# dpeerlab/segger

Hardware: AMD Instinct MI355X
Metric: edges scored/sec (tx->cell) fwd+bwd (higher is better)
Workload: dtype bf16; 1 GPU; C2: single Xenium-scale tile per GPU, 1000000 tx, 10000 nuclei, k=15 kNN (Ett=15000000, Etb=393796, Ep=2435646), training step fwd+bwd+Adam, attention dropout 0.2; parallelism=dp1

## Files before the change

include/segger_amd.h:

```cpp
#ifndef SEGGER_AMD_H
#define SEGGER_AMD_H

#include <stddef.h>
#include <stdint.h>

#ifdef __cplusplus
extern "C" {
#endif

#if defined(__GNUC__) || defined(__clang__)
#pragma GCC visibility push(default)
#endif

#define SEGGER_ABI_VERSION 32

enum segger_status {
  SEGGER_OK = 0,
  SEGGER_EINVAL = -1,
  SEGGER_EUNSUPPORTED = -2,
  SEGGER_EHIP = -3,
  SEGGER_EWORKSPACE = -4
};

enum segger_dtype { SEGGER_F32 = 0, SEGGER_BF16 = 1, SEGGER_F16 = 2 };
// ... 90 lines not shown
  int64_t ld_gxr;
  float* grad_att;
  float* grad_bias;
  void* workspace;
  size_t workspace_bytes;
  const uint8_t* keep_bits_dst;
  const uint8_t* keep_bits_src;
  int32_t src_unique;
  void* zero_rows_out;
  int64_t ld_zero;
  int32_t grad_xl_zeroed;
  int32_t passes;
} segger_gatv2_bwd_args;

size_t segger_gatv2_bwd_workspace_bytes(int64_t n_dst, int32_t heads, int32_t channels);
int segger_gatv2_bwd(const segger_gatv2_bwd_args* args, segger_stream_t stream);
int segger_gatv2_bwd_pair(const segger_gatv2_bwd_args* a, const segger_gatv2_bwd_args* b, segger_stream_t stream);
int segger_dropout_bits(const int32_t* eid, int64_t n_edges, int32_t heads, float dropout_p, const uint64_t* seeds,
                        int32_t n_seeds, const uint64_t* seed_dev, uint8_t* bits, int64_t plane_stride,
                        segger_stream_t stream);
typedef struct segger_bits_job {
  const int32_t* eid;
  int64_t n_edges;
  const uint64_t* seeds;
  int32_t n_seeds;
  int32_t reserved_;
  uint8_t* bits;
  int64_t plane_stride;
} segger_bits_job;
int segger_dropout_bits_many(const segger_bits_job* jobs, int32_t n_jobs, int32_t heads, float dropout_p,
// ... 458 lines not shown
```

segger_amd/_lib.py:

```python
from __future__ import annotations

import ctypes as C
import os
from typing import Optional

import torch

_HERE = os.path.dirname(os.path.abspath(__file__))
LIB_PATH = os.environ.get("SEGGER_AMD_LIB") or os.path.join(_HERE, "libsegger_amd.so")
ABI_VERSION = 32
THRESHOLDS_CHUNK = 1024
FEATURES_TILE, FEATURES_SLAB_ROWS, FEATURES_MAX_SLABS = 64, 512, 32
FEATURES_MAX_COLS, FEATURES_MAX_K = 32768, 256
KNN_BF_MAX_D, KNN_BF_MAX_K, KNN_BF_MAX_SLABS = 256, 64, 32
CONTAM_MAX_TYPES, CONTAM_MAX_K, CONTAM_MAX_REF_GENES, CONTAM_LDS_BYTES = 256, 64, 32768, 65536
MORPH_MAX_VERTS, MORPH_COLS, MORPH_ERR_OFFSETS, MORPH_ERR_CAP = 4096, 12, 1, 2
PJOIN_CONTAINS, PJOIN_INTERSECTS = 0, 1
PJOIN_ERR_OFFSETS, PJOIN_ERR_CAP, PJOIN_ERR_BUFFER, PJOIN_ERR_FILL = 1, 2, 4, 8
BOUNDARY_MAX_SMOOTHING, BOUNDARY_CHUNK_MAX_HULL, BOUNDARY_COUNTERS = 6, 2048, 8
OUTLINE_MAX_POINTS, OUTLINE_COUNTERS = 2048, 10

SEGGER_F32, SEGGER_BF16, SEGGER_F16 = 0, 1, 2
DTYPE_CODE = {torch.float32: SEGGER_F32, torch.bfloat16: SEGGER_BF16, torch.float16: SEGGER_F16}

# ... 187 lines not shown
class WgradArgs(C.Structure):
    _fields_ = [("dy", vp), ("ld_dy", C.c_int64), ("x", vp), ("ld_x", C.c_int64), ("w_t", vp), ("n_rows", C.c_int64),
                ("m_out", C.c_int32), ("reserved_", C.c_int32), ("grad_w", vp), ("grad_b", vp), ("dx", vp),
                ("ld_dx", C.c_int64), ("workspace", vp), ("workspace_bytes", C.c_size_t)]


EXPORTS = {
    "segger_abi_version": (C.c_int, []),
    "segger_csr_block_tables": (C.c_int, [vp, vp, vp, C.c_int64, C.c_int64, vp, vp, vp, vp, vp]),
    "segger_last_error": (C.c_char_p, []),
    "segger_csr_from_coo_workspace_bytes": (C.c_size_t, [C.c_int64, C.c_int64]),
    "segger_csr_from_coo": (C.c_int, [vp, vp, C.c_int64, C.c_int64, C.c_int64, vp, vp, vp, vp, vp, C.c_size_t, vp]),
    "segger_csr_row_order": (C.c_int, [vp, C.c_int64, C.c_int32, vp, vp]),
    "segger_gatv2_fwd": (C.c_int, [C.POINTER(GatFwdArgs), vp]),
    "segger_gatv2_bwd_workspace_bytes": (C.c_size_t, [C.c_int64, C.c_int32, C.c_int32]),
    "segger_gatv2_bwd": (C.c_int, [C.POINTER(GatBwdArgs), vp]),
    "segger_dropout_bits": (C.c_int, [vp, C.c_int64, C.c_int32, C.c_float, vp, C.c_int32, vp, vp, C.c_int64, vp]),
    "segger_gatv2_has_specialised": (C.c_int, [C.c_int32, C.c_int32]),
    "segger_coo_unique": (C.c_int, [vp, C.c_int64, C.c_int64, vp, vp, vp]),
    "segger_stage": (C.c_int, [C.POINTER(StageSeg), C.c_int32, vp]),
    "segger_adam_step": (C.c_int, [C.POINTER(AdamTensor), C.c_int32, C.c_double, C.c_double, C.c_double, C.c_double, vp]),
    "segger_adam_step_ex": (C.c_int, [C.POINTER(AdamTensor), C.c_int32, C.c_double, C.c_double, C.c_double, C.c_double, C.c_int32, vp, C.c_int64, vp]),
    "segger_adam_step_dev": (C.c_int, [C.POINTER(AdamTensor), C.c_int32, vp, C.c_int32, vp, C.c_int64, vp]),
    "segger_transpose_many": (C.c_int, [C.POINTER(TransposeSeg), C.c_int32, vp]),
    "segger_posmlp_supported": (C.c_int, [C.c_int32, C.c_int32, C.c_int32]),
    "segger_posmlp_fwd": (C.c_int, [vp, vp, vp, vp, C.c_int64, C.c_float, C.c_float, vp, vp, vp, vp, vp, vp, vp, vp, vp,
                                    C.c_int32, C.c_int32, vp]),
    "segger_posmlp_wgrad": (C.c_int, [vp, C.c_int64, vp, C.c_int64, C.c_float, C.c_int32, vp, vp, vp, C.c_size_t, vp]),
    "segger_sample_negatives": (C.c_int, [vp, C.c_int64, C.c_int64, vp, C.c_uint64, vp, vp, vp]),
    "segger_edge_cos_argmax": (C.c_int, [C.POINTER(EdgeArgmaxArgs), vp]),
# ... 217 lines not shown
```

segger_amd/csrc/common.h:

```cpp
#pragma once
#include <hip/hip_runtime.h>
#include <stdint.h>
#include <stdio.h>
#include <stdarg.h>
#include "../../include/segger_amd.h"

namespace segger {

void set_error(const char* fmt, ...);
int hip_fail(hipError_t e, const char* what);

#define SEGGER_REQUIRE(cond, ...)                 \
  do {                                            \
    if (!(cond)) {                                \
      ::segger::set_error(__VA_ARGS__);           \
      return SEGGER_EINVAL;                       \
    }                                             \
  } while (0)

#define SEGGER_HIP(call)                                        \
  do {                                                          \
    hipError_t _e = (call);                                     \
    if (_e != hipSuccess) return ::segger::hip_fail(_e, #call); \
  } while (0)
// ... 46 lines not shown
int plan_fwd(const FwdRequest& q, FwdPlan* plan);
int launch_fwd_f32(const FwdRequest& q, const FwdPlan& plan, hipStream_t stream);
int launch_fwd_f32_split(const FwdRequest& q, const FwdPlan& plan, hipStream_t stream);

size_t wgrad_f32_workspace_bytes(int64_t n_rows, int m_out, int k_in);
bool wgrad_f32_split_shape_ok(int m, int k);
int64_t wgrad_f32_split_grid(int64_t n_rows, int m, int k);
int wgrad_f32_split_launch(const float* dy, int64_t ld_dy, const float* x, int64_t ld_x, int64_t n_rows, int m_out, int k_in,
                           float* partial, int64_t* n_slabs, hipStream_t stream);
int wgrad_f32_launch(const void* dy, int64_t ld_dy, const void* x, int64_t ld_x, int64_t n_rows, int m_out, int k_in,
                     float* partial, int64_t* n_slabs, hipStream_t stream);

struct ReduceSeg {
  const float* partial; int64_t n_slabs; int64_t width; int64_t split; float* out0; float* out1;
  float* scratch;
};
constexpr int kReduceGroups = 32;
bool defer_reduce(const ReduceSeg& seg, hipStream_t stream);

constexpr int kWave = 64;
constexpr int kNumXcd = 8;

struct bf16_t { uint16_t v; };
struct f16_t  { uint16_t v; };

#ifdef SEGGER_SCALAR_PAIRS
struct f32x2 {
  float x, y;
};
__device__ __forceinline__ f32x2 operator+(f32x2 a, f32x2 b) { return f32x2{a.x + b.x, a.y + b.y}; }
// ... 160 lines not shown
```

segger_amd/csrc/gatv2.hip:

```cpp
#include "gatv2_launch.h"
#include "draws.h"
#include "post_common.h"

namespace segger {

constexpr int kSlabSplits = 128;

__global__ __launch_bounds__(256) void slab_reduce_stage1(const float* __restrict__ slab, int64_t nblocks, int width,
                                                         float* __restrict__ part) {
  __shared__ float sm[4][64];
  const int lane = threadIdx.x & 63, wave = threadIdx.x >> 6;
  const int colx = blockIdx.x * 64 + lane;
  const int64_t per = (nblocks + kSlabSplits - 1) / kSlabSplits;
  const int64_t r0 = (int64_t)blockIdx.y * per;
  const int64_t r1 = r0 + per < nblocks ? r0 + per : nblocks;
  float s = 0.f;
  if (colx < width)
    for (int64_t r = r0 + wave; r < r1; r += 4) s += slab[r * width + colx];
  sm[wave][lane] = s;
  __syncthreads();
  if (wave == 0 && colx < width) part[(int64_t)blockIdx.y * width + colx] = sm[0][lane] + sm[1][lane] + sm[2][lane] + sm[3][lane];
}

__global__ __launch_bounds__(256) void slab_reduce_stage2(const float* __restrict__ part, int width, int hc,
                                                         float* __restrict__ grad_att, float* __restrict__ grad_bias) {
  const int colx = blockIdx.x * 256 + threadIdx.x;
  if (colx >= width) return;
  float t = 0.f;
  for (int r = 0; r < kSlabSplits; ++r) t += part[(int64_t)r * width + colx];
  if (colx < hc) grad_att[colx] = t;
  else if (grad_bias) grad_bias[colx - hc] = t;
}

// ... 126 lines not shown
                   use_wave_per_row(b->by_dst) && !a->alpha && !b->alpha;
  if (!one) {
    if (!ea) CHECK_RC(launch(Pass::Fwd, pa, a->dtype, a->heads, a->channels, use_wave_per_row(a->by_dst), (hipStream_t)stream));
    if (!eb) CHECK_RC(launch(Pass::Fwd, pb, b->dtype, b->heads, b->channels, use_wave_per_row(b->by_dst), (hipStream_t)stream));
    return SEGGER_OK;
  }
  switch (a->dtype) {
    case SEGGER_F32:  return gatv2_launch_fwd_pair_f32(pa, pb, a->heads, a->channels, (hipStream_t)stream);
    case SEGGER_BF16: return gatv2_launch_fwd_pair_bf16(pa, pb, a->heads, a->channels, (hipStream_t)stream);
    case SEGGER_F16:  return gatv2_launch_fwd_pair_f16(pa, pb, a->heads, a->channels, (hipStream_t)stream);
  }
  set_error("gatv2: unknown dtype %d", a->dtype);
  return SEGGER_EINVAL;
}

extern "C" size_t segger_gatv2_bwd_workspace_bytes(int64_t n_dst, int32_t heads, int32_t channels) {
  if (n_dst <= 0 || heads <= 0 || channels <= 0) return 16;
  const int64_t per = 4 * (int64_t)bwd_row_iters(n_dst);
  const int64_t blocks = (n_dst + per - 1) / per + kNumXcd;
  return (size_t)(blocks + kSlabSplits) * 2 * heads * channels * sizeof(float);
}

namespace {
struct BwdState {
  GatParams p;
  bool direct = false, specialised = false;
  int64_t n_dst = 0, n_src = 0, n_edges = 0;
};

int bwd_prepare(const segger_gatv2_bwd_args* a, BwdState& s) {
  SEGGER_REQUIRE(a != nullptr, "segger_gatv2_bwd: args is NULL");
  SEGGER_REQUIRE(a->heads > 0 && a->channels > 0, "segger_gatv2_bwd: heads/channels must be positive");
  const int hc = a->heads * a->channels;
  const bool specialised = gatv2_has_specialised(a->heads, a->channels);
  g_need_align = specialised;
  CHECK_RC(check_csr("by_dst", a->by_dst));
  const bool direct = a->src_unique != 0;
  SEGGER_REQUIRE(!direct || specialised, "segger_gatv2_bwd: src_unique needs a specialised (heads, channels) geometry");
  if (!direct) {
    CHECK_RC(check_csr("by_src", a->by_src));
    SEGGER_REQUIRE(a->by_dst.n_edges == a->by_src.n_edges && a->by_dst.n_rows == a->by_src.n_cols &&
                   a->by_dst.n_cols == a->by_src.n_rows, "segger_gatv2_bwd: by_dst and by_src describe different graphs");
// ... 5 lines not shown
  if (n_dst > 0) {
    CHECK_RC(check_rows("x_r", a->x_r, a->ld_xr, a->dtype, hc));
    CHECK_RC(check_rows("grad_out", a->grad_out, a->ld_go, a->dtype, hc));
    CHECK_RC(check_rows("pre", a->pre, a->ld_pre, a->dtype, hc));
    CHECK_RC(check_rows("grad_pre", a->grad_pre, a->ld_gp, a->dtype, hc));
    CHECK_RC(check_rows("grad_xr", a->grad_xr, a->ld_gxr, a->dtype, hc));
    SEGGER_REQUIRE(a->lse && a->dsum, "segger_gatv2_bwd: lse / dsum is NULL");
  }
  if (n_src > 0) {
    CHECK_RC(check_rows("x_l", a->x_l, a->ld_xl, a->dtype, hc));
    CHECK_RC(check_rows("grad_xl", a->grad_xl, a->ld_gxl, a->dtype, hc));
  }
  SEGGER_REQUIRE(!(a->dropout_p > 0.f) || n_edges == 0 ||
                     ((a->by_dst.eid || a->keep_bits_dst) && (direct || a->by_src.eid || a->keep_bits_src)),
                 "segger_gatv2_bwd: eid arrays (or keep_bits) are required for dropout");
  const size_t need = segger_gatv2_bwd_workspace_bytes(n_dst, a->heads, a->channels);
  if (a->workspace == nullptr || a->workspace_bytes < need) {
    set_error("segger_gatv2_bwd: workspace %zu < %zu bytes", a->workspace_bytes, need);
    return SEGGER_EWORKSPACE;
  }
  SEGGER_REQUIRE(!a->zero_rows_out || (!direct && specialised),
                 "segger_gatv2_bwd: zero_rows_out needs the two-pass backward of a specialised geometry");
  if (a->zero_rows_out && n_src > 0) CHECK_RC(check_rows("zero_rows_out", a->zero_rows_out, a->ld_zero, a->dtype, hc));

  s.direct = direct; s.specialised = specialised; s.n_dst = n_dst; s.n_src = n_src; s.n_edges = n_edges;
  GatParams& p = s.p;
  p = GatParams{};
  p.xl = a->x_l; p.ld_xl = a->ld_xl; p.xr = a->x_r; p.ld_xr = a->ld_xr;
  p.att = a->att; p.bias = a->bias;
  p.pre = const_cast<void*>(a->pre); p.ld_pre = a->ld_pre; p.lse = const_cast<float*>(a->lse);
  p.gout = a->grad_out; p.ld_go = a->ld_go; p.gpre = a->grad_pre; p.ld_gp = a->ld_gp; p.dsum = a->dsum;
  p.gxl = a->grad_xl; p.ld_gxl = a->ld_gxl; p.gxr = a->grad_xr; p.ld_gxr = a->ld_gxr;
  p.slab = static_cast<float*>(a->workspace);
  p.slope = a->negative_slope; p.apply_gelu = a->apply_gelu;
  set_dropout(p, a->dropout_p, a->seed, a->seed_dev);
  return SEGGER_OK;
}

void bwd_dst_params(const segger_gatv2_bwd_args* a, BwdState& s) {
  GatParams& p = s.p;
  p.indptr = a->by_dst.indptr; p.col = a->by_dst.col; p.eid = a->by_dst.eid; p.order = a->by_dst.row_order;
  p.n_rows = s.n_dst; p.n_edges = s.n_edges; p.rows_per_wave_iter = bwd_row_iters(s.n_dst);
  p.bits = a->keep_bits_dst;
  p.direct_gxl = s.direct ? 1 : 0;
  p.zero_rows = nullptr; p.ld_zero = 0;
}

void bwd_src_params(const segger_gatv2_bwd_args* a, BwdState& s) {
// ... 6 lines not shown
}

int bwd_zero_fill(const segger_gatv2_bwd_args* a, const BwdState& s, hipStream_t stream) {
  const size_t es = esize(a->dtype);
  const int64_t pieces = (int64_t)a->heads * a->channels * es / 16, total = s.n_src * pieces;
  hipLaunchKernelGGL(zero_rows_kernel, dim3((unsigned)((total + 255) / 256)), dim3(256), 0, stream,
                     static_cast<char*>(a->grad_xl), (int64_t)a->ld_gxl * (int64_t)es, pieces, total);
  SEGGER_LAUNCH_CHECK("zero_rows_kernel");
  return SEGGER_OK;
}

int bwd_reduce_slab(const segger_gatv2_bwd_args* a, const BwdState& s, hipStream_t stream) {
  if (!s.specialised) return SEGGER_OK;
  const GatParams& p = s.p;
  const int hc = a->heads * a->channels, width = 2 * hc;
  float* part = p.slab + p.nblocks * width;
  if (defer_reduce(ReduceSeg{p.slab, p.nblocks, width, hc, a->grad_att, a->grad_bias, part}, stream)) return SEGGER_OK;
  hipLaunchKernelGGL(slab_reduce_stage1, dim3((width + 63) / 64, kSlabSplits), dim3(256), 0, stream,
                     p.slab, p.nblocks, width, part);
  hipLaunchKernelGGL(slab_reduce_stage2, dim3((width + 255) / 256), dim3(256), 0, stream,
                     part, width, hc, a->grad_att, a->grad_bias);
  SEGGER_LAUNCH_CHECK("slab_reduce kernels");
  return SEGGER_OK;
}

int bwd_no_destinations(const segger_gatv2_bwd_args* a, hipStream_t stream) {
  const int hc = a->heads * a->channels;
  SEGGER_HIP(hipMemsetAsync(a->grad_att, 0, hc * sizeof(float), stream));
  if (a->grad_bias) SEGGER_HIP(hipMemsetAsync(a->grad_bias, 0, hc * sizeof(float), stream));
  return SEGGER_OK;
}

int64_t bwd_pair_max_rows() {
  static const int64_t v = [] {
    const char* e = getenv("SEGGER_BWD_PAIR_MAX_ROWS");
    return e ? (int64_t)atoll(e) : (int64_t)SEGGER_BWD_PAIR_MAX_ROWS;
// ... 1 lines not shown
  return v;
}
}

extern "C" int segger_gatv2_bwd(const segger_gatv2_bwd_args* a, segger_stream_t stream_) {
  hipStream_t stream = (hipStream_t)stream_;
  BwdState s;
  CHECK_RC(bwd_prepare(a, s));
  SEGGER_REQUIRE(a->passes >= 0 && a->passes <= 3, "segger_gatv2_bwd: passes must be 0 (both), 1 (destination), 2 (source) or 3");
  if (a->passes != 2) {
    bwd_dst_params(a, s);
    if (s.direct && s.n_src > 0 && !a->grad_xl_zeroed) CHECK_RC(bwd_zero_fill(a, s, stream));
    if (s.n_dst > 0) {
      GenericOut gen; gen.grad_att = a->grad_att; gen.grad_bias = a->grad_bias;
      CHECK_RC(launch(Pass::BwdDst, s.p, a->dtype, a->heads, a->channels, use_wave_per_row(a->by_dst), stream, gen));
      if (a->passes != 3) CHECK_RC(bwd_reduce_slab(a, s, stream));
    } else {
      CHECK_RC(bwd_no_destinations(a, stream));
    }
  }
  if (s.direct || a->passes == 1 || a->passes == 3) return SEGGER_OK;
  bwd_src_params(a, s);
  if (s.n_src > 0) CHECK_RC(launch(Pass::BwdSrc, s.p, a->dtype, a->heads, a->channels, use_wave_per_row(a->by_src), stream));
  return SEGGER_OK;
}

extern "C" int segger_gatv2_bwd_pair(const segger_gatv2_bwd_args* a, const segger_gatv2_bwd_args* b, segger_stream_t stream_) {
  hipStream_t stream = (hipStream_t)stream_;
  BwdState sa, sb;
  CHECK_RC(bwd_prepare(a, sa));
  CHECK_RC(bwd_prepare(b, sb));
  const bool zero_by_a = a->zero_rows_out ? (a->zero_rows_out == b->grad_xl && a->ld_zero == b->ld_gxl && b->grad_xl_zeroed)
                                          : !b->grad_xl_zeroed;
  const bool one = !sa.direct && sb.direct && a->dtype == b->dtype && a->heads == b->heads && a->channels == b->channels &&
                   sa.specialised && sa.n_dst > 0 && sa.n_src > 0 && sb.n_dst > 0 && sb.n_src > 0 && sa.n_dst == sb.n_src &&
                   !use_wave_per_row(a->by_dst) && !use_wave_per_row(a->by_src) && use_wave_per_row(b->by_dst) &&
                   zero_by_a && sa.n_src <= bwd_pair_max_rows();
  if (!one) {
    CHECK_RC(segger_gatv2_bwd(a, stream_));
    return segger_gatv2_bwd(b, stream_);
  }
  bwd_dst_params(a, sa);
  sa.p.zero_rows = b->grad_xl; sa.p.ld_zero = b->ld_gxl;
  CHECK_RC(launch(Pass::BwdDst, sa.p, a->dtype, a->heads, a->channels, false, stream));
  CHECK_RC(bwd_reduce_slab(a, sa, stream));
  bwd_src_params(a, sa);
  sa.p.zero_rows = nullptr; sa.p.ld_zero = 0;
  bwd_dst_params(b, sb);
  switch (a->dtype) {
    case SEGGER_F32:  CHECK_RC(gatv2_launch_bwd_src_dst_pair_f32(sa.p, sb.p, a->heads, a->channels, stream)); break;
    case SEGGER_BF16: CHECK_RC(gatv2_launch_bwd_src_dst_pair_bf16(sa.p, sb.p, a->heads, a->channels, stream)); break;
    case SEGGER_F16:  CHECK_RC(gatv2_launch_bwd_src_dst_pair_f16(sa.p, sb.p, a->heads, a->channels, stream)); break;
    default: set_error("gatv2: unknown dtype %d", a->dtype); return SEGGER_EINVAL;
  }
  return bwd_reduce_slab(b, sb, stream);
}

extern "C" int segger_gatv2_has_specialised(int32_t heads, int32_t channels) {
  return gatv2_has_specialised(heads, channels) ? 1 : 0;
}

extern "C" int segger_dropout_bits(const int32_t* eid, int64_t n_edges, int32_t heads, float dropout_p,
                                   const uint64_t* seeds, int32_t n_seeds, const uint64_t* seed_dev, uint8_t* bits,
                                   int64_t plane_stride, segger_stream_t stream) {
  SEGGER_REQUIRE(n_edges >= 0 && heads > 0 && heads <= 8, "segger_dropout_bits: heads must be in 1..8");
  SEGGER_REQUIRE(n_seeds > 0 && n_seeds <= 16 && seeds, "segger_dropout_bits: 1..16 seeds");
  SEGGER_REQUIRE(dropout_p >= 0.f && dropout_p < 1.f, "segger_dropout_bits: dropout_p must be in [0,1)");
  if (n_edges == 0) return SEGGER_OK;
  SEGGER_REQUIRE(eid && bits, "segger_dropout_bits: NULL pointer");
// ... 62 lines not shown
```

segger_amd/csrc/gatv2_kernels.h:

```cpp
#pragma once
#include "common.h"

namespace segger {

#ifndef SEGGER_FWD_UNROLL
#define SEGGER_FWD_UNROLL 4
#endif
#ifndef SEGGER_FWD_UNROLL_WPR
#define SEGGER_FWD_UNROLL_WPR 2
#endif
#ifndef SEGGER_DST_UNROLL
#define SEGGER_DST_UNROLL 4
#endif
#ifndef SEGGER_SRC_UNROLL
#define SEGGER_SRC_UNROLL 4
#endif

#ifndef SEGGER_FWD_WAVES
#define SEGGER_FWD_WAVES 4
#endif
#ifndef SEGGER_BWD_DST_WAVES
#define SEGGER_BWD_DST_WAVES 3
#endif
#ifndef SEGGER_BWD_SRC_WAVES
// ... 24 lines not shown
  const void* xl; int64_t ld_xl;
  const void* xr; int64_t ld_xr;
  const float* att;
  const float* bias;
  void* out; int64_t ld_out;
  void* pre; int64_t ld_pre;
  float* lse;
  float* alpha;
  const void* gout; int64_t ld_go;
  void* gpre; int64_t ld_gp;
  float* dsum;
  void* zero_rows; int64_t ld_zero;
  void* gxl; int64_t ld_gxl;
  void* gxr; int64_t ld_gxr;
  float* slab;
  float slope;
  float drop_scale;
  uint32_t drop_thr;
  uint32_t seed_lo, seed_hi;
  const uint64_t* seed_dev;
  uint64_t seed_raw;
  int32_t apply_gelu;
  int32_t direct_gxl;
  int32_t rows_per_wave_iter;
  int64_t nblocks, nblocks_padded;
};

template <int N, typename F>
__device__ __forceinline__ void static_for(F&& f) {
  if constexpr (N > 0) {
// ... 455 lines not shown
  const LaneGeo L = lane_geo<G>();
  const int h = L.h, ch0 = L.ch0;
  const bool head_leader = L.lane_on && (L.gl % LPH) == 0;
  const char* __restrict__ xl = static_cast<const char*>(p.xl) + (size_t)ch0 * sizeof(T);
  const uint32_t ld_xl = (uint32_t)(p.ld_xl * sizeof(T));
  const bool dropout = p.drop_thr != 0;
  uint32_t seed_lo = p.seed_lo, seed_hi = p.seed_hi;
  if (dropout && p.seed_dev) {
    const uint64_t mixed = splitmix64(p.seed_raw + *p.seed_dev);
    seed_lo = (uint32_t)mixed; seed_hi = (uint32_t)(mixed >> 32);
  }
  constexpr int RPW = WPR ? 1 : NG;
  char* __restrict__ gxl_base = static_cast<char*>(p.gxl) + (size_t)ch0 * sizeof(T);
  const uint32_t ld_gxl = (uint32_t)(p.ld_gxl * sizeof(T));

  f32x2 a1[4], na1[4], a2[4], Pt[4], Qt[4], dbias[4];
  load_att(p.att, ch0, p.slope, kLog2e, a1, a2);
#pragma unroll
  for (int i = 0; i < 4; ++i) { na1[i] = -a1[i]; Pt[i] = splat(0.f); Qt[i] = splat(0.f); dbias[i] = splat(0.f); }

#pragma unroll 1
  for (int it = 0; it < p.rows_per_wave_iter; ++it) {
    const int64_t rbase = ((blk * (int64_t)p.rows_per_wave_iter + it) * 4 + L.wave) * RPW;
    if (rbase >= p.n_rows) break;
    const int64_t pos = rbase + (WPR ? 0 : L.grp);
    const bool row_ok = pos < p.n_rows;
    const int row = visit_row<WPR>(p.order, pos, row_ok);
    int ch0r = L.ch0;
    asm volatile("" : "+v"(ch0r));
    const int ch0 = ch0r;

    f32x2 nxr[4], g[4], Sg[4];
    float D = 0.f, lse = 0.f, Sde = 0.f;
    int64_t beg = 0, end = 0;
// ... 54 lines not shown
        float a_eff = a;
        if constexpr (META != kMetaNone) {
          const bool keep = META == kMetaBits ? (ed[u] & hbit) != 0
                                              : dropout_keep((uint32_t)ed[u], H, h, seed_lo, seed_hi, p.drop_thr);
          da = keep ? da * p.drop_scale : 0.f;
          a_eff = keep ? a * p.drop_scale : 0.f;
        }
        const float de = a * (da - D);
        Sde += de;
        const float nde = -de;
        const f32x2 nde2 = splat(nde);
        f32x2 gx[4];
#pragma unroll
        for (int i = 0; i < 4; ++i) {
          const f32x2 sg = f32x2{sign_mul(nde, nt[i].x), sign_mul(nde, nt[i].y)};
          Pt[i] = pk_fma(nde2, nt[i], Pt[i]);
          Qt[i] = pk_fma(-sg, nt[i], Qt[i]);
          Sg[i] = Sg[i] + sg;
          if constexpr (DIRECT)
            gx[i] = pk_fma(splat(a_eff), g[i], (a1[i] * de + a2[i] * sg) * kLn2);
        }
        if constexpr (DIRECT) {
          if (valid[u] && L.lane_on)
            store_pairs(reinterpret_cast<T*>(gxl_base + (uint64_t)(uint32_t)nbr[u] * ld_gxl), gx);
        }
      }
    };
    if (dropout && p.bits)
      walk_row<GS, WPR, kMetaBits, U>(p.col, p.bits, beg, end, L.lane, L.grp, L.gl, body);
    else if (dropout)
      walk_row<GS, WPR, kMetaEid, U>(p.col, p.eid, beg, end, L.lane, L.grp, L.gl, body);
    else
      walk_row<GS, WPR, kMetaNone, U>(p.col, nullptr, beg, end, L.lane, L.grp, L.gl, body);

    if constexpr (WPR) {
#pragma unroll
      for (int off = GS; off < 64; off <<= 1) {
        Sde += __shfl_xor(Sde, off, 64);
#pragma unroll
        for (int i = 0; i < 4; ++i) {
          Sg[i].x += __shfl_xor(Sg[i].x, off, 64);
          Sg[i].y += __shfl_xor(Sg[i].y, off, 64);
        }
      }
    }
    if (writer) {
      f32x2 dxr[4];
#pragma unroll
      for (int i = 0; i < 4; ++i) dxr[i] = (a1[i] * Sde + a2[i] * Sg[i]) * kLn2;
      store_pairs(static_cast<T*>(p.gxr) + row * p.ld_gxr + ch0, dxr);
    }
  }

  const float c1 = 0.5f * (1.f + p.slope), c2 = 0.5f * (1.f - p.slope);
  float datt[8], db[8];
#pragma unroll
  for (int i = 0; i < 4; ++i) {
    datt[2 * i] = c1 * Pt[i].x + c2 * Qt[i].x; datt[2 * i + 1] = c1 * Pt[i].y + c2 * Qt[i].y;
    db[2 * i] = dbias[i].x; db[2 * i + 1] = dbias[i].y;
  }
#pragma unroll
  for (int off = GS; off < 64; off <<= 1) {
#pragma unroll
    for (int k = 0; k < 8; ++k) {
      datt[k] += __shfl_xor(datt[k], off, 64);
      db[k] += __shfl_xor(db[k], off, 64);
    }
  }
  if (L.grp == 0 && L.lane_on) {
#pragma unroll
    for (int k = 0; k < 8; ++k) { red[L.wave][0][ch0 + k] = datt[k]; red[L.wave][1][ch0 + k] = db[k]; }
  }
  __syncthreads();
  for (int i = threadIdx.x; i < 2 * HC; i += 256) {
    const int which = i / HC, c = i % HC;
    p.slab[blk * (2 * HC) + i] = red[0][which][c] + red[1][which][c] + red[2][which][c] + red[3][which][c];
  }
}

template <typename T, int H, int LPH, bool WPR, bool DIRECT>
__global__ __launch_bounds__(256, DIRECT ? 2 : SEGGER_BWD_DST_WAVES) void gatv2_bwd_dst_kernel(GatParams p) {
  gatv2_bwd_dst_body<T, H, LPH, WPR, DIRECT>(p, blockIdx.x);
}

template <typename T, int H, int LPH, bool WPR>
__device__ __forceinline__ void gatv2_bwd_src_body(SEGGER_BODY_PARAM p, int64_t bid) {
  using G = Geo<H, LPH>;
  constexpr int GS = G::GS, NG = G::NG, U = SEGGER_SRC_UNROLL < GS ? SEGGER_SRC_UNROLL : GS;
  const int64_t blk = xcd_remap(bid, p.nblocks_padded, p.nblocks);
  if (blk < 0) return;
  const LaneGeo L = lane_geo<G>();
  const int h = L.h, ch0 = L.ch0;
  const int64_t pos = WPR ? (blk * 4 + L.wave) : ((blk * 4 + L.wave) * NG + L.grp);
  const bool row_ok = pos < p.n_rows;
  const int row = visit_row<WPR>(p.order, pos, row_ok);
  const char* __restrict__ xr_base = static_cast<const char*>(p.xr) + (size_t)ch0 * sizeof(T);
  const char* __restrict__ g_base = static_cast<const char*>(p.gpre) + (size_t)ch0 * sizeof(T);
  const uint32_t ld_xr = (uint32_t)(p.ld_xr * sizeof(T)), ld_gp = (uint32_t)(p.ld_gp * sizeof(T));
  const bool dropout = p.drop_thr != 0;
  uint32_t seed_lo = p.seed_lo, seed_hi = p.seed_hi;
  if (dropout && p.seed_dev) {
    const uint64_t mixed = splitmix64(p.seed_raw + *p.seed_dev);
    seed_lo = (uint32_t)mixed; seed_hi = (uint32_t)(mixed >> 32);
  }

  f32x2 a1[4], na1[4], a2[4], nv[4], acc[4], Sg[4];
#pragma unroll
  for (int i = 0; i < 4; ++i) { nv[i] = splat(0.f); acc[i] = splat(0.f); Sg[i] = splat(0.f); }
  float Sde = 0.f;
  int64_t beg = 0, end = 0;
  if (row_ok) { beg = p.indptr[row]; end = p.indptr[row + 1]; }
  if (__all(beg == end)) {
    if (row_ok && L.lane_on && (!WPR || L.grp == 0)) {
      store_pairs(static_cast<T*>(p.gxl) + row * p.ld_gxl + ch0, acc);
      if (p.zero_rows) store_pairs(static_cast<T*>(p.zero_rows) + row * p.ld_zero + ch0, acc);
    }
    return;
  }
  load_att(p.att, ch0, p.slope, kLog2e, a1, a2);
#pragma unroll
  for (int i = 0; i < 4; ++i) na1[i] = -a1[i];
  if (row_ok) {
    f32x2 v[4];
    load_pairs(static_cast<const T*>(p.xl) + row * p.ld_xl + ch0, v);
#pragma unroll
    for (int i = 0; i < 4; ++i) nv[i] = neg_canon_zero(v[i]);
  }

  const int hbit = 1 << h;
  auto body = [&](auto meta_c, const bool (&valid)[U], const int (&nbr)[U], const int (&ed)[U]) {
    constexpr int META = decltype(meta_c)::value;
// ... 31 lines not shown
      const float nde = -de;
#pragma unroll
      for (int i = 0; i < 4; ++i) {
        acc[i] = pk_fma(ae2, g[i], acc[i]);
        Sg[i] = Sg[i] + f32x2{sign_mul(nde, nt[i].x), sign_mul(nde, nt[i].y)};
      }
    }
  };
  if (dropout && p.bits)
    walk_row<GS, WPR, kMetaBits, U>(p.col, p.bits, beg, end, L.lane, L.grp, L.gl, body);
  else if (dropout)
    walk_row<GS, WPR, kMetaEid, U>(p.col, p.eid, beg, end, L.lane, L.grp, L.gl, body);
  else
    walk_row<GS, WPR, kMetaNone, U>(p.col, nullptr, beg, end, L.lane, L.grp, L.gl, body);

#pragma unroll
  for (int i = 0; i < 4; ++i) acc[i] = acc[i] + (a1[i] * Sde + a2[i] * Sg[i]) * kLn2;
  if constexpr (WPR) {
#pragma unroll
    for (int off = GS; off < 64; off <<= 1) {
#pragma unroll
      for (int i = 0; i < 4; ++i) {
        acc[i].x += __shfl_xor(acc[i].x, off, 64);
        acc[i].y += __shfl_xor(acc[i].y, off, 64);
      }
    }
  }
  if (row_ok && L.lane_on && (!WPR || L.grp == 0)) {
    store_pairs(static_cast<T*>(p.gxl) + row * p.ld_gxl + ch0, acc);
    if (p.zero_rows) {
// ... 21 lines not shown
```

segger_amd/csrc/reduce.hip:

```cpp
#include "common.h"
#include <mutex>

namespace segger {
namespace {

constexpr int kMaxSegs = 56;
constexpr int64_t kOnePassSlabs = 128;

struct ReduceBatch { int n; ReduceSeg seg[kMaxSegs]; };
static ReduceBatch g_batch;
static bool g_active = false;
static int g_device = -1;
static hipStream_t g_stream = nullptr;
static bool g_stream_set = false;
static std::mutex g_mu;

__global__ __launch_bounds__(256) void reduce_many_kernel(ReduceBatch b) {
  const ReduceSeg g = b.seg[blockIdx.y];
  const int64_t e = (int64_t)blockIdx.x * 256 + threadIdx.x;
  if (e >= g.width) return;
  const float* __restrict__ p = g.partial + e;
  float s0 = 0.f, s1 = 0.f, s2 = 0.f, s3 = 0.f;
  int64_t s = 0;
  for (; s + 3 < g.n_slabs; s += 4) {
    s0 += p[s * g.width];       s1 += p[(s + 1) * g.width];
    s2 += p[(s + 2) * g.width]; s3 += p[(s + 3) * g.width];
  }
  for (; s < g.n_slabs; ++s) s0 += p[s * g.width];
  const float t = (s0 + s1) + (s2 + s3);
  if (e < g.split) g.out0[e] = t;
  else if (g.out1) g.out1[e - g.split] = t;
}

__global__ __launch_bounds__(256) void reduce_many_fold_kernel(ReduceBatch b) {
  const ReduceSeg g = b.seg[blockIdx.y];
  const int64_t e = (int64_t)blockIdx.x * 256 + threadIdx.x;
  if (e >= g.width) return;
  const float* __restrict__ p = g.partial + e;
  const int grp = blockIdx.z;
  float s0 = 0.f, s1 = 0.f, s2 = 0.f, s3 = 0.f;
  int64_t s = grp;
  for (; s + 3 * kReduceGroups < g.n_slabs; s += 4 * kReduceGroups) {
    s0 += p[s * g.width];                       s1 += p[(s + kReduceGroups) * g.width];
    s2 += p[(s + 2 * kReduceGroups) * g.width]; s3 += p[(s + 3 * kReduceGroups) * g.width];
  }
  for (; s < g.n_slabs; s += kReduceGroups) s0 += p[s * g.width];
  g.scratch[(int64_t)grp * g.width + e] = (s0 + s1) + (s2 + s3);
}

}

bool defer_reduce(const ReduceSeg& seg, hipStream_t stream) {
  std::lock_guard<std::mutex> lock(g_mu);
  if (!g_active || g_batch.n >= kMaxSegs || (seg.n_slabs > kOnePassSlabs && seg.scratch == nullptr)) return false;
  int dev = -1;
  if (hipGetDevice(&dev) != hipSuccess || dev != g_device) return false;
  if (!g_stream_set) { g_stream = stream; g_stream_set = true; }
  else if (stream != g_stream) return false;
  g_batch.seg[g_batch.n++] = seg;
  return true;
}

}

using namespace segger;

extern "C" int segger_reductions_defer_begin(void) {
  std::lock_guard<std::mutex> lock(g_mu);
  SEGGER_REQUIRE(!g_active, "segger_reductions_defer_begin: already deferring (flush first)");
// ... 11 lines not shown

extern "C" int segger_reductions_flush(segger_stream_t stream) {
  std::lock_guard<std::mutex> lock(g_mu);
  SEGGER_REQUIRE(g_active, "segger_reductions_flush: nothing is being deferred");
  g_active = false;
  if (g_batch.n == 0) return SEGGER_OK;
  if (g_stream_set && g_stream != (hipStream_t)stream) {
    g_batch.n = 0;
    set_error("segger_reductions_flush: the queued sums were produced on another stream than the one given");
    return SEGGER_EINVAL;
  }
  ReduceBatch longs; longs.n = 0;
  int64_t long_width = 0;
  for (int i = 0; i < g_batch.n; ++i) {
    ReduceSeg& g = g_batch.seg[i];
    if (g.n_slabs <= kOnePassSlabs) continue;
    longs.seg[longs.n++] = g;
    long_width = g.width > long_width ? g.width : long_width;
    g.partial = g.scratch; g.n_slabs = kReduceGroups;
  }
  if (longs.n > 0) {
    hipLaunchKernelGGL(reduce_many_fold_kernel, dim3((unsigned)((long_width + 255) / 256), (unsigned)longs.n, kReduceGroups),
                       dim3(256), 0, (hipStream_t)stream, longs);
    if (hipGetLastError() != hipSuccess) { g_batch.n = 0; set_error("reduce_many_fold_kernel: launch failed"); return SEGGER_EHIP; }
  }
  int64_t width = 0;
  for (int i = 0; i < g_batch.n; ++i) width = g_batch.seg[i].width > width ? g_batch.seg[i].width : width;
  hipLaunchKernelGGL(reduce_many_kernel, dim3((unsigned)((width + 255) / 256), (unsigned)g_batch.n), dim3(256), 0,
                     (hipStream_t)stream, g_batch);
  g_batch.n = 0;
  SEGGER_LAUNCH_CHECK("reduce_many_kernel");
  return SEGGER_OK;
}
```

segger_amd/ops/_common.py:

```python
from __future__ import annotations

import functools
from typing import Optional, Tuple

import torch
from torch import Tensor

from .. import _lib


def _rows(t: Tensor, width: int, name: str) -> Tuple[int, int]:
    sh = t.shape
    if len(sh) != 2 or sh[1] != width:
        raise ValueError(f"{name}: expected [n, {width}], got {tuple(sh)}")
    st = t.stride()
    if sh[0] > 1:
        if st[1] != 1:
            raise ValueError(f"{name}: last dimension must be contiguous")
        return t.data_ptr(), st[0]
    return t.data_ptr(), max(width, st[0])


def _grad_rows(g: Tensor, dt) -> Tensor:
    if g.dtype != dt:
# ... 11 lines not shown
    if torch.is_grad_enabled() and y.requires_grad:
        z._segger_prenorm = (y, float(eps))
    return z


def _prenorm_of(z: Tensor):
    return getattr(z, "_segger_prenorm", None)


@functools.lru_cache(maxsize=None)
def _has_specialised(heads: int, channels: int) -> bool:
    return bool(_lib.load().segger_gatv2_has_specialised(heads, channels))


@functools.lru_cache(maxsize=4096)
def _gat_bwd_ws_bytes(n_dst: int, heads: int, channels: int) -> int:
    return int(_lib.load().segger_gatv2_bwd_workspace_bytes(n_dst, heads, channels))


@functools.lru_cache(maxsize=4096)
def _wgrad_ws_bytes(n: int, m: int, k: int) -> int:
    return int(_lib.load().segger_linear_wgrad_workspace_bytes(n, m, k))


def _seed_parts(seed):
    if isinstance(seed, tuple):
        value, dev = seed
        return int(value) & 0xFFFFFFFFFFFFFFFF, (None if dev is None else dev.data_ptr())
    return int(seed) & 0xFFFFFFFFFFFFFFFF, None


def _bits_ptr(bits: Tensor, n_edges: int) -> int:
# ... 64 lines not shown
```

segger_amd/ops/gatv2.py:

```python
from __future__ import annotations

import ctypes as C
from typing import Optional, Tuple

import torch
from torch import Tensor

from .. import _lib
from .._lib import DTYPE_CODE
from .. import graph as _graph
from ..graph import EdgeCSR, EdgeGraph
from .. import ops
from ._common import _bits_ptr, _defer_keep, _f32_vec, _gat_bwd_ws_bytes, _grad_rows, _has_specialised, _rows, _seed_parts


def gatv2_fwd_launch(by_dst: EdgeCSR, xl: Tensor, xr: Tensor, att: Tensor, bias: Optional[Tensor],
                     heads: int, channels: int, out: Tensor, *, pre: Optional[Tensor] = None,
                     lse: Optional[Tensor] = None, alpha: Optional[Tensor] = None,
                     apply_gelu: bool = False, negative_slope: float = 0.2,
                     dropout_p: float = 0.0, seed: int = 0, keep_bits: Optional[Tensor] = None) -> None:
    a, keep = _gat_fwd_args(by_dst, xl, xr, att, bias, heads, channels, out, pre=pre, lse=lse, alpha=alpha,
                            apply_gelu=apply_gelu, negative_slope=negative_slope, dropout_p=dropout_p, seed=seed,
                            keep_bits=keep_bits)
    with _lib.on_device(xl.device):
# ... 106 lines not shown
    a.pre, a.ld_pre = _rows(pre, hc, "pre")
    a.lse = lse.data_ptr()
    if scratch is not None:
        grad_pre, dsum = scratch
    else:
        grad_pre = torch.empty((n_dst, hc), dtype=dt, device=dev)
        dsum = torch.empty((n_dst, heads, 2), dtype=torch.float32, device=dev)
    a.passes = int(passes)
    gatv2_bwd_launch.scratch = (grad_pre, dsum)
    a.grad_pre, a.ld_gp = _rows(grad_pre, hc, "grad_pre")
    a.dsum = dsum.data_ptr()
    a.grad_xl, a.ld_gxl = _rows(grad_xl, hc, "grad_xl")
    a.grad_xr, a.ld_gxr = _rows(grad_xr, hc, "grad_xr")
    gparams = torch.empty((2, hc), dtype=torch.float32, device=dev)
    a.grad_att, a.grad_bias = gparams[0].data_ptr(), gparams[1].data_ptr()
    ws_bytes = _gat_bwd_ws_bytes(n_dst, heads, channels)
    ws = torch.empty(ws_bytes, dtype=torch.uint8, device=dev)
    a.workspace, a.workspace_bytes = ws.data_ptr(), ws_bytes
    _defer_keep(ws, gparams)
    return a, gparams, (vecs, grad_out, grad_pre, dsum, ws), zero_filled


class _GatV2Aggregate(torch.autograd.Function):

    @staticmethod
    def forward(ctx, xl, xr, att, bias, graph: EdgeGraph, heads, channels, apply_gelu,
                negative_slope, dropout_p, seed, want_alpha, keep_bits=None):
        hc = heads * channels
        dev, dt = xl.device, xl.dtype
        n_dst = graph.n_dst
        need_grad = any(ctx.needs_input_grad[:4])
# ... 105 lines not shown
```

Before: 62.10 million edges/s.

## Split GATv2 attention-weight gradient across dst and src backward passes

In the non-direct two-pass backward, the dst pass no longer accumulates the per-edge Pt/Qt products for the attention gradient. Instead it accumulates a per-row term from xr and the row sums, and the src pass adds a matching per-source-row term into a new workspace slab. The slab reduction (deferred and immediate) now sums both slabs, so it runs after the src pass. This removes two packed FMAs per edge-lane from the dst inner loop, at the cost of an extra block reduction with a syncthreads in the src kernel, more workspace, and a reduction that is moved later.

```diff
diff --git a/include/segger_amd.h b/include/segger_amd.h
--- a/include/segger_amd.h
+++ b/include/segger_amd.h
@@ -128,6 +128,8 @@
 } segger_gatv2_bwd_args;
 
 size_t segger_gatv2_bwd_workspace_bytes(int64_t n_dst, int32_t heads, int32_t channels);
+size_t segger_gatv2_bwd_workspace_bytes_two_pass(int64_t n_dst, int64_t n_src, int64_t n_edges, int32_t heads,
+                                                 int32_t channels);
 int segger_gatv2_bwd(const segger_gatv2_bwd_args* args, segger_stream_t stream);
 int segger_gatv2_bwd_pair(const segger_gatv2_bwd_args* a, const segger_gatv2_bwd_args* b, segger_stream_t stream);
 int segger_dropout_bits(const int32_t* eid, int64_t n_edges, int32_t heads, float dropout_p, const uint64_t* seeds,
diff --git a/segger_amd/_lib.py b/segger_amd/_lib.py
--- a/segger_amd/_lib.py
+++ b/segger_amd/_lib.py
@@ -225,6 +225,7 @@
     "segger_csr_row_order": (C.c_int, [vp, C.c_int64, C.c_int32, vp, vp]),
     "segger_gatv2_fwd": (C.c_int, [C.POINTER(GatFwdArgs), vp]),
     "segger_gatv2_bwd_workspace_bytes": (C.c_size_t, [C.c_int64, C.c_int32, C.c_int32]),
+    "segger_gatv2_bwd_workspace_bytes_two_pass": (C.c_size_t, [C.c_int64, C.c_int64, C.c_int64, C.c_int32, C.c_int32]),
     "segger_gatv2_bwd": (C.c_int, [C.POINTER(GatBwdArgs), vp]),
     "segger_dropout_bits": (C.c_int, [vp, C.c_int64, C.c_int32, C.c_float, vp, C.c_int32, vp, vp, C.c_int64, vp]),
     "segger_gatv2_has_specialised": (C.c_int, [C.c_int32, C.c_int32]),
diff --git a/segger_amd/csrc/common.h b/segger_amd/csrc/common.h
--- a/segger_amd/csrc/common.h
+++ b/segger_amd/csrc/common.h
@@ -84,6 +84,7 @@
 struct ReduceSeg {
   const float* partial; int64_t n_slabs; int64_t width; int64_t split; float* out0; float* out1;
   float* scratch;
+  const float* partial2 = nullptr; int32_t n_slabs2 = 0; int32_t width2 = 0;
 };
 constexpr int kReduceGroups = 32;
 bool defer_reduce(const ReduceSeg& seg, hipStream_t stream);
diff --git a/segger_amd/csrc/gatv2.hip b/segger_amd/csrc/gatv2.hip
--- a/segger_amd/csrc/gatv2.hip
+++ b/segger_amd/csrc/gatv2.hip
@@ -7,6 +7,7 @@
 constexpr int kSlabSplits = 128;
 
 __global__ __launch_bounds__(256) void slab_reduce_stage1(const float* __restrict__ slab, int64_t nblocks, int width,
+                                                         const float* __restrict__ slab2, int64_t nblocks2, int width2,
                                                          float* __restrict__ part) {
   __shared__ float sm[4][64];
   const int lane = threadIdx.x & 63, wave = threadIdx.x >> 6;
@@ -17,6 +18,19 @@
   float s = 0.f;
   if (colx < width)
     for (int64_t r = r0 + wave; r < r1; r += 4) s += slab[r * width + colx];
+  if (colx < width2) {
+    const int64_t per2 = (nblocks2 + kSlabSplits - 1) / kSlabSplits;
+    const int64_t q0 = (int64_t)blockIdx.y * per2;
+    const int64_t q1 = q0 + per2 < nblocks2 ? q0 + per2 : nblocks2;
+    float t[8] = {0.f, 0.f, 0.f, 0.f, 0.f, 0.f, 0.f, 0.f};
+    int64_t r = q0 + wave;
+    for (; r + 28 < q1; r += 32) {
+#pragma unroll
+      for (int k = 0; k < 8; ++k) t[k] += slab2[(r + 4 * k) * width2 + colx];
+    }
+    for (; r < q1; r += 4) t[0] += slab2[r * width2 + colx];
+    s += ((t[0] + t[1]) + (t[2] + t[3])) + ((t[4] + t[5]) + (t[6] + t[7]));
+  }
   sm[wave][lane] = s;
   __syncthreads();
   if (wave == 0 && colx < width) part[(int64_t)blockIdx.y * width + colx] = sm[0][lane] + sm[1][lane] + sm[2][lane] + sm[3][lane];
@@ -173,11 +187,37 @@
   return SEGGER_EINVAL;
 }
 
+namespace {
+struct BwdWorkspace { int64_t dst_cap, src_cap; size_t floats; };
+
+BwdWorkspace bwd_workspace(int64_t n_dst, int64_t n_src, int64_t n_edges, int heads, int channels) {
+  BwdWorkspace w{0, 0, 0};
+  const int64_t hc = (int64_t)heads * channels;
+  if (n_dst > 0) {
+    const int64_t per = 4 * (int64_t)bwd_row_iters(n_dst);
+    w.dst_cap = (n_dst + per - 1) / per + kNumXcd;
+  }
+  if (n_src > 0 && gatv2_has_specialised(heads, channels)) {
+    const int lpr = heads * channels / 8;
+    int gs = 1;
+    while (gs < lpr) gs *= 2;
+    const bool wpr = (double)n_edges / (double)n_src >= kWavePerRowDegree;
+    const int64_t per = wpr ? 4 : 4 * (64 / gs);
+    w.src_cap = (n_src + per - 1) / per + kNumXcd;
+  }
+  w.floats = (size_t)(w.dst_cap + kSlabSplits) * 2 * hc + (size_t)w.src_cap * hc;
+  return w;
+}
+}
+
+extern "C" size_t segger_gatv2_bwd_workspace_bytes_two_pass(int64_t n_dst, int64_t n_src, int64_t n_edges, int32_t heads,
+                                                           int32_t channels) {
+  if ((n_dst <= 0 && n_src <= 0) || heads <= 0 || channels <= 0) return 16;
+  return bwd_workspace(n_dst, n_src, n_edges, heads, channels).floats * sizeof(float);
+}
+
 extern "C" size_t segger_gatv2_bwd_workspace_bytes(int64_t n_dst, int32_t heads, int32_t channels) {
-  if (n_dst <= 0 || heads <= 0 || channels <= 0) return 16;
-  const int64_t per = 4 * (int64_t)bwd_row_iters(n_dst);
-  const int64_t blocks = (n_dst + per - 1) / per + kNumXcd;
-  return (size_t)(blocks + kSlabSplits) * 2 * heads * channels * sizeof(float);
+  return segger_gatv2_bwd_workspace_bytes_two_pass(n_dst, 0, 0, heads, channels);
 }
 
 namespace {
@@ -185,6 +225,8 @@
   GatParams p;
   bool direct = false, specialised = false;
   int64_t n_dst = 0, n_src = 0, n_edges = 0;
+  int64_t dst_blocks = 0, src_blocks = 0;
+  float* part = nullptr;
 };
 
 int bwd_prepare(const segger_gatv2_bwd_args* a, BwdState& s) {
@@ -220,7 +262,8 @@
   SEGGER_REQUIRE(!(a->dropout_p > 0.f) || n_edges == 0 ||
                      ((a->by_dst.eid || a->keep_bits_dst) && (direct || a->by_src.eid || a->keep_bits_src)),
                  "segger_gatv2_bwd: eid arrays (or keep_bits) are required for dropout");
-  const size_t need = segger_gatv2_bwd_workspace_bytes(n_dst, a->heads, a->channels);
+  const BwdWorkspace w = bwd_workspace(n_dst, direct ? 0 : n_src, direct ? 0 : n_edges, a->heads, a->channels);
+  const size_t need = (n_dst > 0 || w.src_cap > 0) ? w.floats * sizeof(float) : 16;
   if (a->workspace == nullptr || a->workspace_bytes < need) {
     set_error("segger_gatv2_bwd: workspace %zu < %zu bytes", a->workspace_bytes, need);
     return SEGGER_EWORKSPACE;
@@ -238,6 +281,8 @@
   p.gout = a->grad_out; p.ld_go = a->ld_go; p.gpre = a->grad_pre; p.ld_gp = a->ld_gp; p.dsum = a->dsum;
   p.gxl = a->grad_xl; p.ld_gxl = a->ld_gxl; p.gxr = a->grad_xr; p.ld_gxr = a->ld_gxr;
   p.slab = static_cast<float*>(a->workspace);
+  p.slab_src = p.slab + w.dst_cap * 2 * hc;
+  s.part = p.slab_src + w.src_cap * hc;
   p.slope = a->negative_slope; p.apply_gelu = a->apply_gelu;
   set_dropout(p, a->dropout_p, a->seed, a->seed_dev);
   return SEGGER_OK;
@@ -274,12 +319,14 @@
   if (!s.specialised) return SEGGER_OK;
   const GatParams& p = s.p;
   const int hc = a->heads * a->channels, width = 2 * hc;
-  float* part = p.slab + p.nblocks * width;
-  if (defer_reduce(ReduceSeg{p.slab, p.nblocks, width, hc, a->grad_att, a->grad_bias, part}, stream)) return SEGGER_OK;
+  const int width2 = s.src_blocks > 0 ? hc : 0;
+  if (defer_reduce(ReduceSeg{p.slab, s.dst_blocks, width, hc, a->grad_att, a->grad_bias, s.part, p.slab_src,
+                             (int32_t)s.src_blocks, width2}, stream))
+    return SEGGER_OK;
   hipLaunchKernelGGL(slab_reduce_stage1, dim3((width + 63) / 64, kSlabSplits), dim3(256), 0, stream,
-                     p.slab, p.nblocks, width, part);
+                     p.slab, s.dst_blocks, width, p.slab_src, s.src_blocks, width2, s.part);
   hipLaunchKernelGGL(slab_reduce_stage2, dim3((width + 255) / 256), dim3(256), 0, stream,
-                     part, width, hc, a->grad_att, a->grad_bias);
+                     s.part, width, hc, a->grad_att, a->grad_bias);
   SEGGER_LAUNCH_CHECK("slab_reduce kernels");
   return SEGGER_OK;
 }
@@ -311,14 +358,19 @@
     if (s.n_dst > 0) {
       GenericOut gen; gen.grad_att = a->grad_att; gen.grad_bias = a->grad_bias;
       CHECK_RC(launch(Pass::BwdDst, s.p, a->dtype, a->heads, a->channels, use_wave_per_row(a->by_dst), stream, gen));
-      if (a->passes != 3) CHECK_RC(bwd_reduce_slab(a, s, stream));
+      s.dst_blocks = s.p.nblocks;
+      if (s.direct || a->passes == 1) CHECK_RC(bwd_reduce_slab(a, s, stream));
     } else {
       CHECK_RC(bwd_no_destinations(a, stream));
     }
   }
   if (s.direct || a->passes == 1 || a->passes == 3) return SEGGER_OK;
   bwd_src_params(a, s);
-  if (s.n_src > 0) CHECK_RC(launch(Pass::BwdSrc, s.p, a->dtype, a->heads, a->channels, use_wave_per_row(a->by_src), stream));
+  if (s.n_src > 0) {
+    CHECK_RC(launch(Pass::BwdSrc, s.p, a->dtype, a->heads, a->channels, use_wave_per_row(a->by_src), stream));
+    s.src_blocks = s.p.nblocks;
+  }
+  if (a->passes == 0 && s.n_dst > 0) CHECK_RC(bwd_reduce_slab(a, s, stream));
   return SEGGER_OK;
 }
 
@@ -340,7 +392,7 @@
   bwd_dst_params(a, sa);
   sa.p.zero_rows = b->grad_xl; sa.p.ld_zero = b->ld_gxl;
   CHECK_RC(launch(Pass::BwdDst, sa.p, a->dtype, a->heads, a->channels, false, stream));
-  CHECK_RC(bwd_reduce_slab(a, sa, stream));
+  sa.dst_blocks = sa.p.nblocks;
   bwd_src_params(a, sa);
   sa.p.zero_rows = nullptr; sa.p.ld_zero = 0;
   bwd_dst_params(b, sb);
@@ -350,6 +402,8 @@
     case SEGGER_F16:  CHECK_RC(gatv2_launch_bwd_src_dst_pair_f16(sa.p, sb.p, a->heads, a->channels, stream)); break;
     default: set_error("gatv2: unknown dtype %d", a->dtype); return SEGGER_EINVAL;
   }
+  sa.src_blocks = sa.p.nblocks; sb.dst_blocks = sb.p.nblocks;
+  CHECK_RC(bwd_reduce_slab(a, sa, stream));
   return bwd_reduce_slab(b, sb, stream);
 }
 
diff --git a/segger_amd/csrc/gatv2_kernels.h b/segger_amd/csrc/gatv2_kernels.h
--- a/segger_amd/csrc/gatv2_kernels.h
+++ b/segger_amd/csrc/gatv2_kernels.h
@@ -62,6 +62,7 @@
   void* gxl; int64_t ld_gxl;
   void* gxr; int64_t ld_gxr;
   float* slab;
+  float* slab_src;
   float slope;
   float drop_scale;
   uint32_t drop_thr;
@@ -547,10 +548,13 @@
   char* __restrict__ gxl_base = static_cast<char*>(p.gxl) + (size_t)ch0 * sizeof(T);
   const uint32_t ld_gxl = (uint32_t)(p.ld_gxl * sizeof(T));
 
-  f32x2 a1[4], na1[4], a2[4], Pt[4], Qt[4], dbias[4];
+  f32x2 a1[4], na1[4], a2[4], Pt[4], Qt[4], datt2[4], dbias[4];
   load_att(p.att, ch0, p.slope, kLog2e, a1, a2);
-#pragma unroll
-  for (int i = 0; i < 4; ++i) { na1[i] = -a1[i]; Pt[i] = splat(0.f); Qt[i] = splat(0.f); dbias[i] = splat(0.f); }
+  const float c1 = 0.5f * (1.f + p.slope), c2 = 0.5f * (1.f - p.slope);
+#pragma unroll
+  for (int i = 0; i < 4; ++i) {
+    na1[i] = -a1[i]; Pt[i] = splat(0.f); Qt[i] = splat(0.f); datt2[i] = splat(0.f); dbias[i] = splat(0.f);
+  }
 
 #pragma unroll 1
   for (int it = 0; it < p.rows_per_wave_iter; ++it) {
@@ -635,11 +639,12 @@
 #pragma unroll
         for (int i = 0; i < 4; ++i) {
           const f32x2 sg = f32x2{sign_mul(nde, nt[i].x), sign_mul(nde, nt[i].y)};
-          Pt[i] = pk_fma(nde2, nt[i], Pt[i]);
-          Qt[i] = pk_fma(-sg, nt[i], Qt[i]);
           Sg[i] = Sg[i] + sg;
-          if constexpr (DIRECT)
+          if constexpr (DIRECT) {
+            Pt[i] = pk_fma(nde2, nt[i], Pt[i]);
+            Qt[i] = pk_fma(-sg, nt[i], Qt[i]);
             gx[i] = pk_fma(splat(a_eff), g[i], (a1[i] * de + a2[i] * sg) * kLn2);
+          }
         }
         if constexpr (DIRECT) {
           if (valid[u] && L.lane_on)
@@ -670,14 +675,21 @@
 #pragma unroll
       for (int i = 0; i < 4; ++i) dxr[i] = (a1[i] * Sde + a2[i] * Sg[i]) * kLn2;
       store_pairs(static_cast<T*>(p.gxr) + row * p.ld_gxr + ch0, dxr);
-    }
-  }
-
-  const float c1 = 0.5f * (1.f + p.slope), c2 = 0.5f * (1.f - p.slope);
+      if constexpr (!DIRECT) {
+#pragma unroll
+        for (int i = 0; i < 4; ++i) datt2[i] = datt2[i] - nxr[i] * (splat(c1 * Sde) + Sg[i] * c2);
+      }
+    }
+  }
+
   float datt[8], db[8];
 #pragma unroll
   for (int i = 0; i < 4; ++i) {
-    datt[2 * i] = c1 * Pt[i].x + c2 * Qt[i].x; datt[2 * i + 1] = c1 * Pt[i].y + c2 * Qt[i].y;
+    if constexpr (DIRECT) {
+      datt[2 * i] = c1 * Pt[i].x + c2 * Qt[i].x; datt[2 * i + 1] = c1 * Pt[i].y + c2 * Qt[i].y;
+    } else {
+      datt[2 * i] = datt2[i].x; datt[2 * i + 1] = datt2[i].y;
+    }
     db[2 * i] = dbias[i].x; db[2 * i + 1] = dbias[i].y;
   }
 #pragma unroll
@@ -707,7 +719,7 @@
 template <typename T, int H, int LPH, bool WPR>
 __device__ __forceinline__ void gatv2_bwd_src_body(SEGGER_BODY_PARAM p, int64_t bid) {
   using G = Geo<H, LPH>;
-  constexpr int GS = G::GS, NG = G::NG, U = SEGGER_SRC_UNROLL < GS ? SEGGER_SRC_UNROLL : GS;
+  constexpr int GS = G::GS, NG = G::NG, U = SEGGER_SRC_UNROLL < GS ? SEGGER_SRC_UNROLL : GS, HC = G::HC;
   const int64_t blk = xcd_remap(bid, p.nblocks_padded, p.nblocks);
   if (blk < 0) return;
   const LaneGeo L = lane_geo<G>();
@@ -731,11 +743,30 @@
   float Sde = 0.f;
   int64_t beg = 0, end = 0;
   if (row_ok) { beg = p.indptr[row]; end = p.indptr[row + 1]; }
+  __shared__ float red_src[4][HC];
+  auto block_partial = [&](const f32x2 (&w)[4]) {
+    float d[8];
+#pragma unroll
+    for (int i = 0; i < 4; ++i) { d[2 * i] = w[i].x; d[2 * i + 1] = w[i].y; }
+#pragma unroll
+    for (int off = GS; off < 64; off <<= 1) {
+#pragma unroll
+      for (int k = 0; k < 8; ++k) d[k] += __shfl_xor(d[k], off, 64);
+    }
+    if (L.grp == 0 && L.lane_on) {
+#pragma unroll
+      for (int k = 0; k < 8; ++k) red_src[L.wave][L.ch0 + k] = d[k];
+    }
+    __syncthreads();
+    for (int i = threadIdx.x; i < HC; i += 256)
+      p.slab_src[blk * HC + i] = red_src[0][i] + red_src[1][i] + red_src[2][i] + red_src[3][i];
+  };
   if (__all(beg == end)) {
     if (row_ok && L.lane_on && (!WPR || L.grp == 0)) {
       store_pairs(static_cast<T*>(p.gxl) + row * p.ld_gxl + ch0, acc);
       if (p.zero_rows) store_pairs(static_cast<T*>(p.zero_rows) + row * p.ld_zero + ch0, acc);
     }
+    block_partial(acc);
     return;
   }
   load_att(p.att, ch0, p.slope, kLog2e, a1, a2);
@@ -797,6 +828,13 @@
   else
     walk_row<GS, WPR, kMetaNone, U>(p.col, nullptr, beg, end, L.lane, L.grp, L.gl, body);
 
+  {
+    const float c1 = 0.5f * (1.f + p.slope), c2 = 0.5f * (1.f - p.slope);
+    f32x2 w[4];
+#pragma unroll
+    for (int i = 0; i < 4; ++i) w[i] = -(nv[i] * (splat(c1 * Sde) + Sg[i] * c2));
+    block_partial(w);
+  }
 #pragma unroll
   for (int i = 0; i < 4; ++i) acc[i] = acc[i] + (a1[i] * Sde + a2[i] * Sg[i]) * kLn2;
   if constexpr (WPR) {
diff --git a/segger_amd/csrc/reduce.hip b/segger_amd/csrc/reduce.hip
--- a/segger_amd/csrc/reduce.hip
+++ b/segger_amd/csrc/reduce.hip
@@ -5,6 +5,7 @@
 namespace {
 
 constexpr int kMaxSegs = 56;
+static_assert(sizeof(ReduceSeg) * kMaxSegs + 8 <= 4096, "the table travels as a kernel argument");
 constexpr int64_t kOnePassSlabs = 128;
 
 struct ReduceBatch { int n; ReduceSeg seg[kMaxSegs]; };
@@ -27,6 +28,14 @@
     s2 += p[(s + 2) * g.width]; s3 += p[(s + 3) * g.width];
   }
   for (; s < g.n_slabs; ++s) s0 += p[s * g.width];
+  if (e < g.width2) {
+    const float* __restrict__ q = g.partial2 + e;
+    for (s = 0; s + 3 < g.n_slabs2; s += 4) {
+      s0 += q[s * g.width2];       s1 += q[(s + 1) * g.width2];
+      s2 += q[(s + 2) * g.width2]; s3 += q[(s + 3) * g.width2];
+    }
+    for (; s < g.n_slabs2; ++s) s0 += q[s * g.width2];
+  }
   const float t = (s0 + s1) + (s2 + s3);
   if (e < g.split) g.out0[e] = t;
   else if (g.out1) g.out1[e - g.split] = t;
@@ -45,6 +54,14 @@
     s2 += p[(s + 2 * kReduceGroups) * g.width]; s3 += p[(s + 3 * kReduceGroups) * g.width];
   }
   for (; s < g.n_slabs; s += kReduceGroups) s0 += p[s * g.width];
+  if (e < g.width2) {
+    const float* __restrict__ q = g.partial2 + e;
+    for (s = grp; s + 3 * kReduceGroups < g.n_slabs2; s += 4 * kReduceGroups) {
+      s0 += q[s * g.width2];                       s1 += q[(s + kReduceGroups) * g.width2];
+      s2 += q[(s + 2 * kReduceGroups) * g.width2]; s3 += q[(s + 3 * kReduceGroups) * g.width2];
+    }
+    for (; s < g.n_slabs2; s += kReduceGroups) s0 += q[s * g.width2];
+  }
   g.scratch[(int64_t)grp * g.width + e] = (s0 + s1) + (s2 + s3);
 }
 
@@ -52,7 +69,7 @@
 
 bool defer_reduce(const ReduceSeg& seg, hipStream_t stream) {
   std::lock_guard<std::mutex> lock(g_mu);
-  if (!g_active || g_batch.n >= kMaxSegs || (seg.n_slabs > kOnePassSlabs && seg.scratch == nullptr)) return false;
+  if (!g_active || g_batch.n >= kMaxSegs || ((seg.n_slabs > kOnePassSlabs || seg.n_slabs2 > kOnePassSlabs) && seg.scratch == nullptr)) return false;
   int dev = -1;
   if (hipGetDevice(&dev) != hipSuccess || dev != g_device) return false;
   if (!g_stream_set) { g_stream = stream; g_stream_set = true; }
@@ -94,10 +111,10 @@
   int64_t long_width = 0;
   for (int i = 0; i < g_batch.n; ++i) {
     ReduceSeg& g = g_batch.seg[i];
-    if (g.n_slabs <= kOnePassSlabs) continue;
+    if (g.n_slabs <= kOnePassSlabs && g.n_slabs2 <= kOnePassSlabs) continue;
     longs.seg[longs.n++] = g;
     long_width = g.width > long_width ? g.width : long_width;
-    g.partial = g.scratch; g.n_slabs = kReduceGroups;
+    g.partial = g.scratch; g.n_slabs = kReduceGroups; g.n_slabs2 = 0; g.width2 = 0;
   }
   if (longs.n > 0) {
     hipLaunchKernelGGL(reduce_many_fold_kernel, dim3((unsigned)((long_width + 255) / 256), (unsigned)longs.n, kReduceGroups),
diff --git a/segger_amd/ops/_common.py b/segger_amd/ops/_common.py
--- a/segger_amd/ops/_common.py
+++ b/segger_amd/ops/_common.py
@@ -49,8 +49,8 @@
 
 
 @functools.lru_cache(maxsize=4096)
-def _gat_bwd_ws_bytes(n_dst: int, heads: int, channels: int) -> int:
-    return int(_lib.load().segger_gatv2_bwd_workspace_bytes(n_dst, heads, channels))
+def _gat_bwd_ws_bytes(n_dst: int, n_src: int, n_edges: int, heads: int, channels: int) -> int:
+    return int(_lib.load().segger_gatv2_bwd_workspace_bytes_two_pass(n_dst, n_src, n_edges, heads, channels))
 
 
 @functools.lru_cache(maxsize=4096)
diff --git a/segger_amd/ops/gatv2.py b/segger_amd/ops/gatv2.py
--- a/segger_amd/ops/gatv2.py
+++ b/segger_amd/ops/gatv2.py
@@ -144,7 +144,8 @@
     a.grad_xr, a.ld_gxr = _rows(grad_xr, hc, "grad_xr")
     gparams = torch.empty((2, hc), dtype=torch.float32, device=dev)
     a.grad_att, a.grad_bias = gparams[0].data_ptr(), gparams[1].data_ptr()
-    ws_bytes = _gat_bwd_ws_bytes(n_dst, heads, channels)
+    two_pass = not a.src_unique
+    ws_bytes = _gat_bwd_ws_bytes(n_dst, g.n_src if two_pass else 0, g.n_edges if two_pass else 0, heads, channels)
     ws = torch.empty(ws_bytes, dtype=torch.uint8, device=dev)
     a.workspace, a.workspace_bytes = ws.data_ptr(), ws_bytes
     _defer_keep(ws, gparams)
```

After: 62.83 million edges/s (median of 6 runs). 1.2% higher.
